# zacharielegault/lesion-gnn

Hardware: AMD Instinct MI355X
Metric: graphs/sec (fwd+bwd) on batched k-NN lesion graphs at 1/2/4/8 MI355X (higher is better)
Workload: dtype f32; 1 GPU; C2: 2-layer GCN fwd+CE+bwd+Adam, graph build per forward; step_launch=graph:step, criterion=CE fused with the model node (forward_loss), sync_bn=False, process_group=False, adam=lgnn, graphs_per_gpu=1024, global_batch=1024, nodes=65536, edges=524288, k=8, d_in=128, parallelism=dp1

## Files before the change

include/lgnn.h:

```cpp
#ifndef LGNN_H
#define LGNN_H

#include <stddef.h>
#include <stdint.h>

#ifdef __cplusplus
extern "C" {
#endif

#define LGNN_ABI_VERSION 40

#define LGNN_OK 0
#define LGNN_EINVAL (-22)
#define LGNN_ENOSPC (-28)
#define LGNN_EBUSY (-16)

#define LGNN_SLOT_FLAG0 7
#define LGNN_SLOT_FLAGS 256
#define LGNN_TILE_OPEN_EXTRA (LGNN_SLOT_FLAG0 + LGNN_SLOT_FLAGS)

#define LGNN_LOOPS_KEEP 0
#define LGNN_LOOPS_REMAINING 1
#define LGNN_LOOPS_READD 2

// ... 296 lines not shown
                               float* const* dWp, float* const* dbp, int num_partials,
                               float* dS_ws, int32_t* tile_open, const float* dlogits,
                               const float* Wout, int num_classes, const void* adjt,
                               void* stream);
struct lgnn_ce_src;
int lgnn_gcn_stack_bwd_s3f_ce(const int64_t* batch, const int32_t* gptr, int pool_mean,
                              int64_t num_graphs, const int32_t* rowptr, const int32_t* col,
                              const float* w, const int32_t* tptr, const int32_t* tidx,
                              const float* tw, const float* X, int64_t M, int L,
                              const uint16_t* planes_t, const float* const* W,
                              const float* const* H, const float* const* S, const int* widths,
                              float* const* dWp, float* const* dbp, int num_partials,
                              float* dS_ws, int32_t* tile_open, const struct lgnn_ce_src* ce,
                              const float* Wout, int num_classes, const void* adjt,
                              void* stream);

size_t lgnn_s3_weight_planes_numel(int out_features, int in_features, int planes);
int lgnn_s3_weight_planes(const float* W, int rows, int cols, int transposed, int planes,
                          uint16_t* Wp, void* stream);
#define LGNN_MAX_WPREP 16
int lgnn_s3_weight_planes_multi(int n, const float* const* W, const int* rows, const int* cols,
                                const int* transposed, int planes, uint16_t* const* Wp,
                                void* stream);
int lgnn_s3_gemm(const float* A, int64_t M, int K, const uint16_t* Wp, int N, int planes,
                 const float* bias, float* Y, float* colsum_part, void* stream);
int lgnn_s3_gemm_att(const float* A, int64_t M, int K, const uint16_t* Wp, int N, int planes,
                     float* Y, const float* att_src, const float* att_dst, int heads, int C,
                     float* a_s, float* a_d, void* stream);
int lgnn_s3_wgrad_partials(int64_t M, int K, int N);
int lgnn_s3_wgrad(const float* dY, int N, const float* X, int64_t M, int K, int planes,
// ... 165 lines not shown
```

lesion_gnn_amd/csrc/loss.hip:

```cpp
#include "common.h"

namespace {

constexpr int CT = 1024;

__device__ __forceinline__ float block_sum_fixed(float v, float* red) {
  const int lane = threadIdx.x & 63, wave = threadIdx.x >> 6;
  for (int o = 32; o > 0; o >>= 1) v += __shfl_xor(v, o, 64);
  if (lane == 0) red[wave] = v;
  __syncthreads();
  float t = 0.f;
  if (threadIdx.x == 0) {
    for (int w = 0; w < CT / 64; ++w) t += red[w];
    red[CT / 64] = t;
  }
  __syncthreads();
  return red[CT / 64];
}

template <bool FACTORS>
__global__ __launch_bounds__(CT) void k_ce_fwd(const float* __restrict__ z,
                                               const int64_t* __restrict__ y,
                                               const float* __restrict__ weight, int64_t B, int C,
                                               float* __restrict__ lse, float* __restrict__ loss,
// ... 87 lines not shown
  const float dl = smooth ? fminf(fmaxf(d, -1.f), 1.f) : 2.f * d;
  float g = gloss ? gloss[0] / (float)B * dl : 0.f;
  if (gpred) g += gpred[i];
  dz[i] = (zi >= lo && zi <= hi) ? g : 0.f;
}

struct ReduceJobs {
  CeSrc ce;
  int ce_part[LGNN_MAX_REDUCE];
  const float* part[LGNN_MAX_REDUCE];
  const float* factor[LGNN_MAX_REDUCE];
  float* out[LGNN_MAX_REDUCE];
  int64_t len[LGNN_MAX_REDUCE];
  int P[LGNN_MAX_REDUCE];
  int width[LGNN_MAX_REDUCE];
};

constexpr int RT = 1024;
__global__ __launch_bounds__(RT) void k_reduce_multi(ReduceJobs jobs) {
  __shared__ f32x4 red4[16][64];
  float(*red)[64] = reinterpret_cast<float(*)[64]>(red4);
  const int j = blockIdx.y;
  const int64_t len = jobs.len[j];
  const bool vec = !jobs.factor[j] && !jobs.ce_part[j] && (len & 3) == 0 && len >= 4096;
  if ((int64_t)blockIdx.x * (vec ? 256 : 64) >= len) return;
  const float* __restrict__ part = jobs.part[j];
  int P = jobs.P[j];
  const int lane = threadIdx.x & 63, wave = threadIdx.x >> 6;
  if (vec) {
    const int64_t i4 = (int64_t)blockIdx.x * 256 + 4 * lane;
    const int64_t ic4 = i4 < len ? i4 : len - 4;
    f32x4 s4 = {0.f, 0.f, 0.f, 0.f};
    int p = wave;
    for (; p + 16 * 15 < P; p += 16 * 16) {
      f32x4 v[16];
#pragma unroll
      for (int u = 0; u < 16; ++u) v[u] = ld4(part + (int64_t)(p + 16 * u) * len + ic4);
#pragma unroll
      for (int u = 0; u < 16; ++u) s4 += v[u];
    }
    for (; p < P; p += 16) s4 += ld4(part + (int64_t)p * len + ic4);
    red4[wave][lane] = s4;
    __syncthreads();
// ... 153 lines not shown
                       static_cast<const float*>(target), B, lo, hi, smooth_l1, grad_loss,
                       grad_pred, dz);
  LGNN_LAUNCH_CHECK();
  return LGNN_OK;
}

extern "C" int lgnn_reduce_partials_multi(int n, const float* const* partials,
                                          const int* num_partials, const int64_t* len,
                                          float* const* out, void* stream) {
  return lgnn_reduce_jobs(n, partials, nullptr, nullptr, num_partials, len, out, stream);
}

static int reduce_jobs(int n, const float* const* partials, const float* const* factor,
                       const int* width, const int* num_partials, const int64_t* len,
                       float* const* out, const int* ce_job, const lgnn_ce_src* ce, int C,
                       void* stream) {
  if (n <= 0 || n > LGNN_MAX_REDUCE || !partials || !num_partials || !len || !out)
    return LGNN_EINVAL;
  ReduceJobs jobs = {};
  if (ce_job) {
    if (!ce || !ce->pm || !ce->wt || !ce->wsum || !ce->gloss || C < 1)
      return LGNN_EINVAL;
    jobs.ce = CeSrc{ce->pm, ce->wt, ce->wsum, ce->gloss, C};
  }
  int64_t maxlen = 0;
  for (int j = 0; j < n; ++j) {
    const bool cj = ce_job && ce_job[j];
    if ((!partials[j] && !cj) || !out[j] || num_partials[j] <= 0 || len[j] < 0)
      return LGNN_EINVAL;
    if (cj) {
      const int64_t rows = factor && factor[j] && width ? len[j] / width[j] : len[j];
      if (rows != C) return LGNN_EINVAL;
      jobs.ce_part[j] = 1;
    }
    if (factor && factor[j]) {
      if (!width || width[j] <= 0 || len[j] % width[j] != 0) return LGNN_EINVAL;
      jobs.factor[j] = factor[j];
      jobs.width[j] = width[j];
    }
    jobs.part[j] = partials[j];
    jobs.out[j] = out[j];
    jobs.len[j] = len[j];
    jobs.P[j] = num_partials[j];
    if (len[j] > maxlen) maxlen = len[j];
  }
  if (maxlen == 0) return LGNN_OK;
  hipLaunchKernelGGL(k_reduce_multi, dim3((unsigned)((maxlen + 63) / 64), (unsigned)n), dim3(RT),
                     0, as_stream(stream), jobs);
  LGNN_LAUNCH_CHECK();
  return LGNN_OK;
}

extern "C" int lgnn_reduce_jobs(int n, const float* const* partials, const float* const* factor,
                                const int* width, const int* num_partials, const int64_t* len,
                                float* const* out, void* stream) {
  return reduce_jobs(n, partials, factor, width, num_partials, len, out, nullptr, nullptr, 0,
                     stream);
}

extern "C" int lgnn_reduce_jobs_ce(int n, const float* const* partials,
                                   const float* const* factor, const int* width,
                                   const int* num_partials, const int64_t* len,
                                   float* const* out, const int* ce_job, const lgnn_ce_src* ce,
                                   int num_classes, void* stream) {
  if (!ce_job) return LGNN_EINVAL;
  return reduce_jobs(n, partials, factor, width, num_partials, len, out, ce_job, ce, num_classes,
                     stream);
}
```

lesion_gnn_amd/csrc/node.hip:

```cpp
#include "common.h"
#include "tile.h"

namespace {

constexpr int TM = 64;
constexpr int TN = 128;
constexpr int KC = 128;
constexpr int LDS = KC + 4;
constexpr int NT = 256;
constexpr int CAPE = 1024;
constexpr int EB = 8;

struct TileIdx {
  int rp[TM + 1];
  int col[CAPE];
  float w[CAPE];
};

__device__ __forceinline__ f32x4 zero4() { return f32x4{0.f, 0.f, 0.f, 0.f}; }
__device__ __forceinline__ f32x4 sel4(bool c, f32x4 v) { return c ? v : zero4(); }

template <bool VEC>
__device__ __forceinline__ void fill_direct(float* Xs, const float* __restrict__ X, int64_t M,
                                            int K, int k0, int64_t r0) {
// ... 645 lines not shown
                                    H, act, X, M, K, rowptr, col, w, self_scale, W, N, dXpre,
                                    dW_partial, db_partial, num_partials, nullptr, 0, 0, stream);
}

extern "C" int lgnn_node_linear_bwd_tiles(int grad_mode, const float* dY, const int64_t* batch,
                                          const int32_t* gptr, int pool_mean,
                                          const int32_t* tptr, const int32_t* tidx,
                                          const float* tw, float tself, const float* H, int act,
                                          const float* X, int64_t M, int K,
                                          const int32_t* rowptr, const int32_t* col,
                                          const float* w, float self_scale, const float* W, int N,
                                          float* dXpre, float* dW_partial, float* db_partial,
                                          int num_partials, const int32_t* tile_open,
                                          int want_open, int accumulate, void* stream) {
  if (M < 0 || K <= 0 || N <= 0 || (N & 3) || !W || !dW_partial) return LGNN_EINVAL;
  if (accumulate < 0 || accumulate > 2 ||
      (accumulate == 2 && (!tile_open || num_partials > LGNN_SLOT_FLAGS)))
    return LGNN_EINVAL;
  const bool fast = bwd_fast(M, N, K, rowptr != nullptr);
  if (tile_open && !fast) return LGNN_EINVAL;
  if (!tile_open && num_partials != (fast ? lgnn_tile_partials(M) : grid_partials(M, N, K)))
    return LGNN_EINVAL;
  if (num_partials <= 0) return LGNN_EINVAL;
  if (act != LGNN_ACT_NONE && act != LGNN_ACT_ELU) return LGNN_EINVAL;
  if (act == LGNN_ACT_ELU && !H) return LGNN_EINVAL;
  if (grad_mode == LGNN_GRAD_POOL && (!batch || !gptr)) return LGNN_EINVAL;
  if (grad_mode == LGNN_GRAD_TRANSPOSE && (!tptr || !tidx)) return LGNN_EINVAL;
  if (grad_mode < 0 || grad_mode > 2 || (M > 0 && (!dY || !X))) return LGNN_EINVAL;
  const bool gather = rowptr != nullptr;
  if (gather && (!col || (K & 3))) return LGNN_EINVAL;
  if (fast && M > 0) {
    const hipError_t ef = lgnn_tile_bwd(s_(stream), grad_mode, dY, batch, gptr, pool_mean, tptr,
// ... 64 lines not shown
```

lesion_gnn_amd/csrc/stack3_bwd.hip:

```cpp
#include <cstdlib>
#include "common.h"
#include "tile.h"
#include "tile_util.h"
#include "s3_util.h"
#include "tile_lw.h"

namespace lgnn_s3 {

constexpr int BM_POOL = 0;
constexpr int BM_CONV = 1;
constexpr int BM_LIN = 2;

struct BwdLayerArgs {
  const float* dZin;
  const int64_t* batch;
  const int32_t* gptr;
  int pool_mean;
  int64_t num_graphs;
  const float* Hout;
  const float* Hin;
  const uint16_t* WpT;
  float* dZout;
  float* dWp;
  float* dbp;
// ... 572 lines not shown
        const float wgt = tw[j];
        const int64_t src = tidx[j];
        if (c < N) {
          a0 += wgt * dS[src * N + c];
          a1 += wgt * dS[src * N + c + 1];
        }
      }
      if (c < N) {
        dZ0[row * N + c] = a0;
        dZ0[row * N + c + 1] = a1;
      }
    }
  }
}

template <int NL, bool AG, bool XIN = false>
__global__ __launch_bounds__(NT, 1) void k_s3_fbwd(const int32_t* __restrict__ rowptr,
                                                   const int32_t* __restrict__ col,
                                                   const float* __restrict__ w, int64_t M,
                                                   FBwdArgs a, const int32_t* __restrict__ tmask,
                                                   OpenBwdArgs o) {
  constexpr int L = NL - 1;
  constexpr int ND = XIN ? NL - 1 : NL;
  __shared__ __attribute__((aligned(16))) FBwdSmem sm;
  const int64_t ntiles = (M + TM - 1) / TM;
  float* const scr = reinterpret_cast<float*>(sm.Adj[0]);
  const int NLast = a.width[L + 1];
  const Buf bP = mkbuf(a.dP, a.num_graphs * NLast * 4);

  f32x16 dw[ND][4];
#pragma unroll
  for (int l = 0; l < ND; ++l)
#pragma unroll
    for (int kb = 0; kb < 4; ++kb) dw[l][kb] = f32x16{};
  float dbacc[NL];
#pragma unroll
  for (int l = 0; l < NL; ++l) dbacc[l] = 0.f;

// ... 189 lines not shown
    if (has_next) idx_load_body(R, col, w);
    }
    const bool aexact = __builtin_amdgcn_readfirstlane(sm.flag) == 0;
    STAMP(stamp++);

    f32x16 xp[2];
#pragma unroll
    for (int l = L; l >= 1; --l) {
      const int K = a.width[l];
      const bool elu_prev = l >= 2;
      const bool fold = !XIN && l == 1;
      f32x16 hp[2];
      {
        const int tq = fresh_tid();
        const int h = (tq >> 5) & 1, k = 32 * (tq >> 6) + (tq & 31);
        load_pt(hp, a.H[l - 1], (ABL & 16) ? 0 : M, r0, K, k, K, h);
      }
      {
        float sacc = 0.f;
#pragma unroll
        for (int q = 0; q < 2; ++q)
#pragma unroll
          for (int r = 0; r < 16; ++r) sacc += dz[q][r];
        sacc += __shfl_xor(sacc, 32, 64);
        dbacc[l] += sacc;
      }
      u32x4 dzp[4][3];
      split_p(dz, dzp);
      if (fold && L == 1) {
        const int tq = fresh_tid();
        const int h = (tq >> 5) & 1, k = 32 * (tq >> 6) + (tq & 31);
// ... 55 lines not shown
      if (!fold) {
        const int tq = fresh_tid();
        const int h = (tq >> 5) & 1, li = tq & 31, wv = tq >> 6, qi = li & 3;
#pragma unroll
        for (int q = 0; q < 2; ++q)
#pragma unroll
          for (int j = 0; j < 4; ++j) {
            const int st = 2 * q + (j >> 1), i0 = 2 * (j & 1);
            const int off = ap_off(32 * q + 8 * j + 4 * h + qi, 32 * wv + (li & ~3));
#pragma unroll
            for (int p = 0; p < 3; ++p)
              sts8(sm.Gt[p] + off, quad_transpose_bf16(gp[st][p][i0], gp[st][p][i0 + 1], qi));
          }
      }
      STAMP(stamp++);
      {
        const int tq = fresh_tid();
        const int h = (tq >> 5) & 1, li = tq & 31, k = 32 * (tq >> 6) + li;
#pragma unroll
        for (int q = 0; q < 2; ++q)
#pragma unroll
          for (int gq = 0; gq < 4; ++gq) {
            u32x2 o[3];
            split4(f32x4{hp[q][4 * gq], hp[q][4 * gq + 1], hp[q][4 * gq + 2], hp[q][4 * gq + 3]},
                   o);
            const int off = hf_off(k, 32 * q + 8 * gq + 4 * h);
#pragma unroll
            for (int p = 0; p < 3; ++p) sts8(sm.Img[p] + off, o[p]);
          }
      }
      const uint16_t* wbase;
// ... 46 lines not shown
                nap = adj_split(sm);
              }
              const int t2 = fresh_tid();
              pre_cnt = (has_next && t2 < TM) ? a.gptr[pre_g + 1] - a.gptr[pre_g] : 0;
              if (has_head(a)) {
#pragma unroll
                for (int c = 0; c < kMaxHeadC; ++c)
                  pre_dl[c] = (has_next && t2 < TM && c < a.C) ? head_raw(a, pre_g, c) : 0.f;
                if (a.ce.pm) pre_wt = (has_next && t2 < TM) ? a.ce.wt[pre_g] : 0.f;
              }
            }
#pragma unroll
            for (int kb = 0; kb < 4; ++kb) {
              u32x4 hb[3], xb[3];
              const int off = hf_chunk(32 * kb + li, 2 * s + h);
#pragma unroll
              for (int p = 0; p < 3; ++p) hb[p] = lds16(sm.Img[p] + off);
#pragma unroll
              for (int p = 0; p < 3; ++p) xb[p] = lds16(sm.Gt[p] + off);
              if constexpr (!(ABL & 1)) {
                dw[1][kb] = mfma_s3(gp[s], hb, dw[1][kb]);
                dw[0][kb] = mfma_s3(gp[s], xb, dw[0][kb]);
              }
            }
            S3F_SB();
          }
        }
        lds_barrier();
        if constexpr (AG && kAdjPipe) {
          adj_write(sm, nap);
          lds_barrier();
        }
        STAMP(stamp++);
      } else {
      {
        const int tq = fresh_tid();
// ... 83 lines not shown
            pre_dl[c] = (has_next && tq < TM && c < a.C) ? head_raw(a, pre_g, c) : 0.f;
          if (a.ce.pm) pre_wt = (has_next && tq < TM) ? a.ce.wt[pre_g] : 0.f;
        }
      }
      lds_barrier();
      if constexpr (AG && kAdjPipe) {
        const AdjPlanes nap = adj_split(sm);
        lds_barrier();
        adj_write(sm, nap);
        lds_barrier();
      }
      STAMP(stamp++);
    }
    t = tn;
  }
  if (write_slots) {
    if constexpr (!XIN) {
      unsigned char* const timg = sm.Img[0];
      constexpr int TPL = 2 * TM * AROW;
      static_assert(3 * TPL == sizeof(sm.Img) + sizeof(sm.Gt) && offsetof(FBwdSmem, Gt) ==
                                                                     sizeof(sm.Img), "T image");
      float* const gl = sm.hl;
      lds_barrier();
      {
        const int tq = fresh_tid();
        const int h = (tq >> 5) & 1, li = tq & 31, wv = tq >> 6;
#pragma unroll
        for (int kb = 0; kb < 4; ++kb)
#pragma unroll
          for (int gq = 0; gq < 4; ++gq) {
            u32x2 o3[3];
            split4(f32x4{dw[0][kb][4 * gq], dw[0][kb][4 * gq + 1], dw[0][kb][4 * gq + 2],
// ... 53 lines not shown
        };
        fold_pair(wa, 0);
        load_w2(wa, 2);
        fold_pair(wb, 1);
        load_w2(wb, 3);
        fold_pair(wa, 2);
        fold_pair(wb, 3);
        dbs += __shfl_xor(dbs, 32, 64);
        dbacc[0] = dbs;
      }
      STAMP(stamp++);
    }
    const int tq = threadIdx.x;
    const int h = (tq >> 5) & 1, li = tq & 31, wv = tq >> 6;
#pragma unroll
    for (int l = XIN ? 1 : 0; l < NL; ++l) {
      const int N = a.width[l + 1], K = a.width[l];
      float* slab = a.dWp[l] + (int64_t)blockIdx.x * N * K;
#pragma unroll
      for (int kb = 0; kb < 4; ++kb) {
        const int k = 32 * kb + li;
#pragma unroll
        for (int r = 0; r < 16; ++r) {
          const int n = 32 * wv + (r & 3) + 8 * (r >> 2) + 4 * h;
          if (n < N && k < K) {
            st_wt(slab + (int64_t)n * K + k, dw[XIN ? l - 1 : l][kb][r]);
          }
        }
      }
      const int n = 32 * wv + li;
      if (h == 0 && n < N) a.dbp[l][(int64_t)blockIdx.x * N + n] = dbacc[l];
    }
  }
  if (o.sync && tmask[ntiles] > 0) {
    static_assert(sizeof(LwSmem) <= sizeof(FBwdSmem), "open-tile LDS aliases the fused LDS");
    __syncthreads();
    LwSmem& lw = *reinterpret_cast<LwSmem*>(&sm);
    for (int l = L; l >= 0; --l) {
      if (l < L) grid_sync(o.sync, L - l);
      const int K = a.width[l], N = a.width[l + 1];
      const float* Sx = l == 0 ? a.X : o.S[l - 1];
      if (l == L)
        bwd_tiles<LGNN_GRAD_POOL, LGNN_ACT_ELU, true>(
            lw.A, lw.C, lw.ti, a.dP, a.batch, a.gptr, a.pool_mean, nullptr, nullptr, nullptr, 0.f,
            a.H[l], Sx, M, K, o.W[l], N, o.dS[l & 1], a.dWp[l], a.dbp[l], tmask, 1, 1, a.dlog,
            a.Wout, a.C, BnFuse{}, a.ce);
      else if (l >= 1)
        bwd_tiles<LGNN_GRAD_TRANSPOSE, LGNN_ACT_ELU, true>(
            lw.A, lw.C, lw.ti, o.dS[(l + 1) & 1], a.batch, a.gptr, a.pool_mean, o.tptr, o.tidx,
            o.tw, 0.f, a.H[l], Sx, M, K, o.W[l], N, o.dS[l & 1], a.dWp[l], a.dbp[l], tmask, 1,
            1);
      else if constexpr (XIN)
        open_dz0(a.dZ0, o.dS[1], o.tptr, o.tidx, o.tw, M, N, tmask);
      else
        bwd_tiles<LGNN_GRAD_TRANSPOSE, LGNN_ACT_NONE, false>(
            lw.A, lw.C, lw.ti, o.dS[1], a.batch, a.gptr, a.pool_mean, o.tptr, o.tidx, o.tw, 0.f,
            nullptr, Sx, M, K, o.W[0], N, nullptr, a.dWp[0], a.dbp[0], tmask, 1, 1);
    }
    grid_exit(o.sync);
  }
}

}

static int stack_bwd_s3f(const float* dP, const int64_t* batch, const int32_t* gptr,
                         int pool_mean, int64_t num_graphs, const int32_t* rowptr,
                         const int32_t* col, const float* w, const float* X, int64_t M, int L,
                         const uint16_t* planes_t, const float* const* H, const int* widths,
                         float* const* dWp, float* const* dbp, int num_partials,
                         const int32_t* tile_open, const lgnn_s3::OpenBwdArgs& o, void* stream,
                         const float* dlogits = nullptr, const float* Wout = nullptr,
                         int num_classes = 0, const void* adjt = nullptr,
// ... 89 lines not shown
    if (dlogits || !ce->pm || !ce->wt || !ce->wsum || !ce->gloss)
      return LGNN_EINVAL;
    a.ce = CeSrc{ce->pm, ce->wt, ce->wsum, ce->gloss, num_classes};
  }
  a.Wout = Wout;
  a.C = num_classes;
  a.adjt = static_cast<const unsigned char*>(adjt);
  a.batch = batch;
  a.gptr = gptr;
  a.pool_mean = pool_mean;
  a.num_graphs = num_graphs;
  a.X = X;
  a.WpT = planes_t;
  a.dZ0 = dz0;
  for (int l = 0; l <= L + 1; ++l) a.width[l] = widths[l];
  for (int l = 0; l <= L; ++l) {
    if (!lgnn_tile_fits(M, widths[l], widths[l + 1]) || !H[l] || !dWp[l] || !dbp[l])
      return LGNN_EINVAL;
    a.H[l] = H[l];
    a.dWp[l] = dWp[l];
    a.dbp[l] = dbp[l];
  }
  hipStream_t s = as_stream(stream);
  if (M == 0) {
    for (int l = 0; l <= L; ++l)
      if (hipMemsetAsync(dWp[l], 0, (size_t)widths[l] * widths[l + 1] * 4, s) != hipSuccess ||
          hipMemsetAsync(dbp[l], 0, (size_t)widths[l + 1] * 4, s) != hipSuccess)
        return (int)hipGetLastError();
    return LGNN_OK;
  }
  const dim3 grid((unsigned)num_partials), blk(lgnn_tile::NT);
  if (o.sync) {
    const int cap = lgnn_fused_grid_capacity(1);
    if (cap < (int)grid.x) return cap == LGNN_EINVAL ? cap : cap < 0 ? -cap : LGNN_EBUSY;
  }
  if (L == 3 && adjt)
    hipLaunchKernelGGL((lgnn_s3::k_s3_fbwd<4, true, true>), grid, blk, 0, s, rowptr, col, w, M, a,
                       tile_open, o);
  else if (L == 3)
    hipLaunchKernelGGL((lgnn_s3::k_s3_fbwd<4, false, true>), grid, blk, 0, s, rowptr, col, w, M,
                       a, tile_open, o);
  else if (L == 1 && adjt)
    hipLaunchKernelGGL((lgnn_s3::k_s3_fbwd<2, true>), grid, blk, 0, s, rowptr, col, w, M, a,
                       tile_open, o);
  else if (L == 1)
    hipLaunchKernelGGL((lgnn_s3::k_s3_fbwd<2, false>), grid, blk, 0, s, rowptr, col, w, M, a,
                       tile_open, o);
  else if (adjt)
    hipLaunchKernelGGL((lgnn_s3::k_s3_fbwd<3, true>), grid, blk, 0, s, rowptr, col, w, M, a,
                       tile_open, o);
  else
    hipLaunchKernelGGL((lgnn_s3::k_s3_fbwd<3, false>), grid, blk, 0, s, rowptr, col, w, M, a,
                       tile_open, o);
  const hipError_t e = hipGetLastError();
  return e == hipSuccess ? LGNN_OK : (int)e;
}
// ... 12 lines not shown
```

lesion_gnn_amd/csrc/tile_lw.h:

```cpp
#pragma once
#include <type_traits>

#include "tile_util.h"

namespace lgnn_tile {

template <int UB = EB>
__device__ __forceinline__ f32x4 agg_row_local(const TileIdx& ti, int rr, const float* A) {
  static_assert(UB <= EB, "row batches read at most EB padding entries");
  const int li = threadIdx.x & 31;
  const int eb = ti.rp[0];
  const int e0 = ti.rp[rr] - eb, e1 = ti.rp[rr + 1] - eb;
  f32x4 acc = zero4();
  for (int e = e0; e < e1; e += UB) {
    int2 p[UB];
#pragma unroll
    for (int u = 0; u < UB; ++u) p[u] = ti.ow[e + u];
    f32x4 v[UB];
#pragma unroll
    for (int u = 0; u < UB; ++u) v[u] = ld4(A + p[u].x + 4 * li);
#pragma unroll
    for (int u = 0; u < UB; ++u) {
      const float wv = e + u < e1 ? __int_as_float(p[u].y) : 0.f;
      acc += wv * v[u];
// ... 450 lines not shown
#pragma unroll
              for (int j = 0; j < 4; ++j) {
                const float gg = v[j] * bn_elu_grad(z[j], bsc[j], bsh[j]) * m[j];
                const float xh = (z[j] - bmu[j]) * bis[j];
                s0[j] += (double)gg;
                s1[j] += (double)gg * (double)xh;
              }
            }
          }
        }
      }
    }
    __syncthreads();
  }
  if constexpr (BNM == BN_GSTATS) bn_part_write(reinterpret_cast<double*>(A), s0, s1, bn.part, K);
  const bool skipped = accumulate == 2 && blockIdx.x < LGNN_SLOT_FLAGS &&
                       tmask[ntiles + LGNN_SLOT_FLAG0 + blockIdx.x] != 0;
  if (accumulate && tfirst >= ntiles && !skipped) return;
  const bool add = accumulate && !skipped;
  float* slab = dWp + (int64_t)blockIdx.x * N * K;
#pragma unroll
  for (int j = 0; j < 4; ++j) {
    const int k = 32 * j + li;
#pragma unroll
    for (int r = 0; r < 16; ++r) {
      const int o = 32 * wave + (r & 3) + 8 * (r >> 2) + 4 * h;
      if (o < N && k < K) {
        float* p = slab + (int64_t)o * K + k;
        *p = add ? *p + dw[j][r] : dw[j][r];
      }
    }
  }
  if (dbp && tid < N) {
    float* p = dbp + (int64_t)blockIdx.x * N + tid;
    *p = add ? *p + dbacc : dbacc;
  }
}

}
```

lesion_gnn_amd/ops.py:

```python
from __future__ import annotations

import ctypes
import weakref
from collections import namedtuple
from typing import NamedTuple

import torch
from torch.utils import _pytree as pytree

from . import _lib
from .graph import NO_CSR, Csr, Graph


def _compiling() -> bool:
    return torch.compiler.is_compiling()


def _lgnn():
    from . import library

    return library


def _f32c(t: torch.Tensor) -> torch.Tensor:
# ... 40 lines not shown


STACK_MAX = 8


FUSED_BWD = True
LAZY_TRANSPOSE = True


MFMA_MODE = "s3"
BWD_MODE = "s3f"
BWD_S3 = BWD_MODE in ("s3", "s3f")
OPEN_IN_FUSED = "auto"
OPEN_IN_FUSED_BWD = OPEN_IN_FUSED
HEAD_FOLD = True
_CAPACITY: dict = {}


def fused_grid_capacity(direction: str, dev) -> int:
    key = (direction, torch.device(dev).index)
    cap = _CAPACITY.get(key)
    if cap is None:
        with torch.cuda.device(dev):
            cap = int(_lib.load().lgnn_fused_grid_capacity(0 if direction == "fwd" else 1))
        if cap < 0:
            _lib.check(cap, "lgnn_fused_grid_capacity")
        _CAPACITY[key] = cap
    return cap


# ... 132 lines not shown
        s_out = ss[l - 1] if l > 0 else None
        _lib.call("lgnn_node_linear_fwd_tiles", inp, M, inp.size(1), c.rowptr, c.col, c.w, 0.0,
                  Ws[l], bs[l], Ws[l].size(0),
                  _lib.LGNN_ACT_ELU if l > 0 else _lib.LGNN_ACT_NONE, hs[l], s_out, open_, 1,
                  _s(dev))
    return hs, ss, planes_t, adjt_t


def head_in_stack_bwd(graph: Graph, L: int, C: int, s3: bool) -> bool:
    return (HEAD_FOLD and s3 and BWD_MODE == "s3f" and L <= 3 and C <= 8 and
            _open_in_fused(OPEN_IN_FUSED_BWD, graph, "bwd"))


def stack_bwd(dp: torch.Tensor | None, x: torch.Tensor, graph: Graph, mean: bool, Ws: list,
              hs: list, ss: list, reducer: list, planes_t: torch.Tensor | None = None,
              head: tuple | None = None, kind: str = "gcn", adjt_t: torch.Tensor | None = None):
    csr = graph.csr(kind)
    open_ = graph.tile_open(kind)
    M = x.size(0)
    L = len(Ws) - 1
    dev = x.device
    lib = _lib.load()
    s3 = planes_t is not None
    s3f = s3 and _s3f(L) and (L <= 2 or _open_in_fused(OPEN_IN_FUSED_BWD, graph, "bwd"))
    adjt = (adjt_t if adjt_t is not None else _adjt_ptr(planes_t, L)) if s3f else None
    P = lib.lgnn_gcn_stack_bwd_s3_partials(M) if s3 and not s3f else \
        lib.lgnn_gcn_stack_bwd_partials(M)
    _lib.check(0 if P > 0 else P, "lgnn_gcn_stack_bwd_partials")
    widths = [x.size(1)] + [W.size(0) for W in Ws]
    per = [widths[l + 1] * widths[l] + widths[l + 1] for l in range(L + 1)]
    slab = torch.empty(P * sum(per), dtype=torch.float32, device=dev)
    dWp, dbp, off = [], [], 0
    for l in range(L + 1):
        nk, n = widths[l + 1] * widths[l], widths[l + 1]
        dWp.append(slab[off:off + P * nk])
        dbp.append(slab[off + P * nk:off + P * (nk + n)])
        off += P * (nk + n)
    Sx = [x] + list(ss)
    dlog, W_out = head if head is not None else (None, None)
    ce = dlog if isinstance(dlog, _lib.CeSrc) else None
    B = dp.size(0) if dp is not None else (graph.num_graphs if ce is not None else dlog.size(0))
    if s3f and _open_in_fused(OPEN_IN_FUSED_BWD, graph, "bwd"):
        dS_ws = torch.empty((3 if L == 3 else 2) * M * 128, dtype=torch.float32, device=dev)
        common = (graph.batch, graph.gptr, int(mean), B, csr.rowptr, csr.col, csr.w, csr.tptr,
                  csr.tidx, csr.tw, x, M, L, planes_t, Ws, hs, ss, widths, dWp, dbp, P, dS_ws,
                  open_)
        if ce is not None:
            _lib.call("lgnn_gcn_stack_bwd_s3f_ce", *common, ctypes.byref(ce), W_out,
                      W_out.size(0), adjt, _s(dev))
        else:
            _lib.call("lgnn_gcn_stack_bwd_s3f_all", dp, *common, dlog, W_out,
                      W_out.size(0) if head else 0, adjt, _s(dev))
        if L == 3:
            dz0 = dS_ws[2 * M * 128:2 * M * 128 + M * widths[1]].view(M, widths[1])
            first = dense_wgrad(dz0, x, False, want_db=True, reducer=reducer)
            return [first] + _stack_bwd_outputs(L, widths, dWp, dbp, P, dev, reducer, l0=1)
        return _stack_bwd_outputs(L, widths, dWp, dbp, P, dev, reducer)
    assert head is None, "dP from the logits gradient only in the single-launch split-3 path"
    if s3f:
        _lib.call("lgnn_gcn_stack_bwd_s3f", dp, graph.batch, graph.gptr, int(mean), dp.size(0),
                  csr.rowptr, csr.col, csr.w, x, M, L, planes_t, hs, widths, dWp, dbp, P, open_,
                  adjt, _s(dev))
    elif s3:
        dz_ws = torch.empty(2 * M * 128, dtype=torch.float32, device=dev)
        _lib.call("lgnn_gcn_stack_bwd_s3", dp, graph.batch, graph.gptr, int(mean), dp.size(0),
                  csr.rowptr, csr.col, csr.w, x, M, L, planes_t, hs, widths, dWp, dbp, P, dz_ws,
                  open_, _s(dev))
    else:
        _lib.call("lgnn_gcn_stack_bwd", dp, graph.batch, graph.gptr, int(mean), csr.rowptr,
                  csr.col, csr.w, x, M, L, Ws, hs, widths, dWp, dbp, P, open_, _s(dev))
    dS = None
    for l in reversed(range(L + 1)):
        K, N = widths[l], widths[l + 1]
        if l == L:
            mode, dY, tc = _lib.LGNN_GRAD_POOL, dp, NO_CSR
        else:
            mode, dY, tc = _lib.LGNN_GRAD_TRANSPOSE, dS, csr
        dX = torch.empty(M, K, dtype=torch.float32, device=dev) if l > 0 else None
        _lib.call("lgnn_node_linear_bwd_tiles", mode, dY, graph.batch, graph.gptr, int(mean),
                  tc.tptr, tc.tidx, tc.tw, 0.0, hs[l] if l > 0 else None,
                  _lib.LGNN_ACT_ELU if l > 0 else _lib.LGNN_ACT_NONE, Sx[l], M, K, None, None,
                  None, 0.0, Ws[l], N, dX, dWp[l], dbp[l], P, open_, 1, 2 if s3f else 1,
                  _s(dev))
        dS = dX
    return _stack_bwd_outputs(L, widths, dWp, dbp, P, dev, reducer)


def _stack_bwd_outputs(L, widths, dWp, dbp, P, dev, reducer, l0=0):
    out = []
    for l in range(l0, L + 1):
        dW = torch.empty(widths[l + 1], widths[l], dtype=torch.float32, device=dev)
        db = torch.empty(widths[l + 1], dtype=torch.float32, device=dev)
        reducer.extend([(dWp[l], P, dW.numel(), dW), (dbp[l], P, db.numel(), db)])
        out.append((dW, db))
    return out


def num_partials(M: int, N: int, K: int, gather: bool = False) -> int:
    p = _lib.load().lgnn_bwd_num_partials(M, N, K, int(gather))
    _lib.check(0 if p > 0 else p, "lgnn_bwd_num_partials")
# ... 47 lines not shown

CE_PART = object()


def reduce_multi(jobs: list, dev, ce=None, num_classes: int = 0) -> None:
    for i in range(0, len(jobs), 16):
        chunk = jobs[i:i + 16]
        n = len(chunk)
        is_ce = [j[0] is CE_PART for j in chunk]
        parts = [None if c else j[0] for j, c in zip(chunk, is_ce)]
        nps = [j[1] for j in chunk]
        lens = [j[2] for j in chunk]
        outs = [j[3] for j in chunk]
        fac = [j[4] if len(j) > 4 else None for j in chunk]
        wid = [j[5] if len(j) > 4 else 0 for j in chunk]
        if any(is_ce):
            if ce is None:
                raise _lib.LgnnError("reduce_multi: a CE_PART job needs the CE source")
            _lib.call("lgnn_reduce_jobs_ce", n, parts, fac, wid, nps, lens, outs,
                      [int(c) for c in is_ce], ctypes.byref(ce), int(num_classes), _s(dev))
        elif any(len(j) > 4 for j in chunk):
            _lib.call("lgnn_reduce_jobs", n, parts, fac, wid, nps, lens, outs, _s(dev))
        else:
            _lib.call("lgnn_reduce_partials_multi", n, parts, nps, lens, outs, _s(dev))


def spmm_raw(rowptr, col, w, self_scale: float, x: torch.Tensor) -> torch.Tensor:
    M, D = x.shape
    y = torch.empty_like(x)
    _lib.call("lgnn_spmm", rowptr, col, w, float(self_scale), x, M, D, y, _s(x.device))
    return y
# ... 523 lines not shown
    kind = sv.plan.kind
    csr = graph.csr(kind)
    W_out = params[2 + 2 * L]
    dlogits = _f32c(dlogits) if dlogits is not None else None
    grads = [None] * len(params)
    red: list = []
    if sv.plan.fused_bwd and not want_dx:
        Ws = [params[2 * l] for l in range(L + 1)]
        if head_in_stack_bwd(graph, L, W_out.size(0), sv.planes_t is not None):
            C, D = W_out.shape
            B = pooled.size(0)
            dWo = torch.empty_like(W_out)
            dbo = torch.empty(C, dtype=torch.float32, device=x.device)
            part = CE_PART if ce is not None else dlogits
            red += [(part, B, C * D, dWo, pooled, D), (part, B, C, dbo)]
            outs = stack_bwd(None, x, graph, sv.mean, Ws, hs, ss, red, sv.planes_t,
                             head=(ce[0] if ce is not None else dlogits, W_out), kind=kind,
                             adjt_t=sv.adjt)
        else:
            dp, dWo, dbo = pool_head_bwd(dlogits, pooled, W_out)
            outs = stack_bwd(dp, x, graph, sv.mean, Ws, hs, ss, red, sv.planes_t, kind=kind,
                             adjt_t=sv.adjt)
        grads[2 + 2 * L], grads[3 + 2 * L] = dWo, dbo
        for l, (dW, db) in enumerate(outs):
            grads[2 * l], grads[2 * l + 1] = dW, db
        reduce_multi(red, x.device, ce=ce[0] if ce is not None else None,
                     num_classes=W_out.size(0))
        return None, grads
    assert ce is None, "the CE-formed logits gradient only on the fused head path"
    dp, dWo, dbo = pool_head_bwd(dlogits, pooled, W_out)
    grads[2 + 2 * L], grads[3 + 2 * L] = dWo, dbo
    if sv.plan.fused:
        ss = [spmm_raw(csr.rowptr, csr.col, csr.w, 0.0, hs[l]) for l in range(L)]
    dS = None
    for l in reversed(range(L)):
        W = params[2 + 2 * l]
        if l == L - 1:
            mode, dY, tc = _lib.LGNN_GRAD_POOL, dp, None
        else:
            mode, dY, tc = _lib.LGNN_GRAD_TRANSPOSE, dS, csr
        saved_s = sv.plan.saved_s[l]
        dS, dW, db = linear_bwd(mode, dY, H=hs[l + 1], act=_lib.LGNN_ACT_ELU,
# ... 1447 lines not shown
```

Before: 4.891 million graphs/s.

## Defer in_proj/conv1 weight-grad fold into a post-reduce kernel for shallow GCN

For stacks with at most two conv layers and no saved H[0], the fused backward kernel stops forming the layer-1 weight gradient against H[0] per tile. It instead accumulates a compact T = dZ1ᵀ·X product plus a bias-gradient vector in extra partial slabs. A new fold kernel then reconstructs dW0, db0 and dW1 from T, W0, b0 and W1 once after the partial reduction, and a live flag lets the reduction skip or zero jobs. The aim is to drop the per-tile H[0] loads and MFMA work and to avoid materialising H[0]. The cost is an extra slab, an extra launch and more complex reduction and control logic.

After: 5.118 million graphs/s, median of 6. 4.6% higher.

```diff
diff --git a/include/lgnn.h b/include/lgnn.h
--- a/include/lgnn.h
+++ b/include/lgnn.h
@@ -334,6 +334,15 @@
                               float* dS_ws, int32_t* tile_open, const struct lgnn_ce_src* ce,
                               const float* Wout, int num_classes, const void* adjt,
                               void* stream);
+
+int lgnn_gcn_fold_wgrad(const float* T, const float* g, const float* W0, const float* b0,
+                        const float* W1, int d_in, int w1, int w2, const float* dW0_open,
+                        const float* db0_open, const float* dW1_open, const int32_t* live,
+                        float* dW0, float* db0, float* dW1, void* stream);
+int lgnn_reduce_jobs_live(int n, const float* const* partials, const float* const* factor,
+                          const int* width, const int* num_partials, const int64_t* len,
+                          float* const* out, const int* ce_job, const struct lgnn_ce_src* ce,
+                          int num_classes, const int32_t* const* live, void* stream);
 
 size_t lgnn_s3_weight_planes_numel(int out_features, int in_features, int planes);
 int lgnn_s3_weight_planes(const float* W, int rows, int cols, int transposed, int planes,
diff --git a/lesion_gnn_amd/csrc/foldgrad.hip b/lesion_gnn_amd/csrc/foldgrad.hip
--- /dev/null
+++ b/lesion_gnn_amd/csrc/foldgrad.hip
@@ -0,0 +1,153 @@
+#include "common.h"
+
+namespace {
+
+constexpr int FT = 256;
+constexpr int FR = 8;
+constexpr int FW = 128;
+constexpr int FLD = FW + 4;
+
+struct FoldArgs {
+  const float* T;
+  const float* g;
+  const float* W0;
+  const float* b0;
+  const float* W1;
+  const float* dW0_open;
+  const float* db0_open;
+  const float* dW1_open;
+  const int32_t* live;
+  float* dW0;
+  float* db0;
+  float* dW1;
+  int d_in, w1, w2;
+};
+
+__device__ __forceinline__ void copy_load(f32x4 (&v)[16], const float* src, int n4) {
+#pragma unroll
+  for (int u = 0; u < 16; ++u) {
+    const int f = threadIdx.x + u * FT;
+    v[u] = ld4(src + 4 * (int64_t)(f < n4 ? f : 0));
+  }
+}
+__device__ __forceinline__ void copy_store(float* dst, int ld, const f32x4 (&v)[16], int n4,
+                                           int q) {
+  int r = threadIdx.x / q, p = threadIdx.x - r * q;
+  const int dr = FT / q, dp = FT - dr * q;
+#pragma unroll
+  for (int u = 0; u < 16; ++u) {
+    if ((int)threadIdx.x + u * FT < n4) st4(dst + r * ld + 4 * p, v[u]);
+    r += dr;
+    p += dp;
+    if (p >= q) {
+      p -= q;
+      ++r;
+    }
+  }
+}
+
+__global__ __launch_bounds__(FT) void k_fold_wgrad(FoldArgs a) {
+  __shared__ __attribute__((aligned(16))) float big[FW * FLD];
+  __shared__ __attribute__((aligned(16))) float strip[FW * FR];
+  __shared__ float gs[FW];
+  const int t = threadIdx.x;
+  const int c = t & (FW - 1), rg = t >> 7;
+  const int d_in = a.d_in, w1 = a.w1, w2 = a.w2;
+  const int nb0 = (w1 + FR - 1) / FR;
+  const int q = d_in / 4;
+  const f32x4 z = {0.f, 0.f, 0.f, 0.f};
+  const bool role0 = (int)blockIdx.x < nb0;
+  const int r0 = FR * (role0 ? (int)blockIdx.x : (int)blockIdx.x - nb0);
+  const int rows = role0 ? w1 : w2, cols = role0 ? d_in : w1;
+  float* const out = role0 ? a.dW0 : a.dW1;
+  const float* const open = role0 ? a.dW0_open : a.dW1_open;
+  f32x4 v[16];
+  copy_load(v, role0 ? a.T : a.W0, (role0 ? w2 : w1) * q);
+  const bool alive = !a.live || a.live[0] != 0;
+  if (!alive && open == out && (!role0 || a.db0_open == a.db0)) return;
+  float ov[4] = {0.f, 0.f, 0.f, 0.f};
+  if (open && c < cols) {
+#pragma unroll
+    for (int j = 0; j < 4; ++j)
+      if (r0 + 4 * rg + j < rows) ov[j] = open[(int64_t)(r0 + 4 * rg + j) * cols + c];
+  }
+  const bool dbt = role0 && t < FR && r0 + t < w1;
+  const float obv = (a.db0_open && dbt) ? a.db0_open[r0 + t] : 0.f;
+  float acc[4] = {0.f, 0.f, 0.f, 0.f};
+  double dbs = 0.0;
+  if (alive) {
+    const float gv = t < w2 ? a.g[t] : 0.f;
+    if (role0) {
+      const int sn = t >> 1, si = r0 + 4 * (t & 1);
+      const f32x4 sv = (sn < w2 && si < w1) ? ld4(a.W1 + (int64_t)sn * w1 + si) : z;
+      copy_store(big, d_in, v, w2 * q, q);
+      st4(strip + FR * sn + 4 * (t & 1), sv);
+      if (t < FW) gs[t] = gv;
+      __syncthreads();
+      const int kc = c < d_in ? c : 0;
+#pragma unroll 8
+      for (int n = 0; n < w2; ++n) {
+        const float tv = big[n * d_in + kc];
+        const f32x4 wv = ld4(strip + FR * n + 4 * rg);
+#pragma unroll
+        for (int j = 0; j < 4; ++j) acc[j] = fmaf(wv[j], tv, acc[j]);
+      }
+      if (dbt) {
+        double s4[4] = {0.0, 0.0, 0.0, 0.0};
+        for (int n = 0; n < w2; n += 4) {
+#pragma unroll
+          for (int e = 0; e < 4; ++e)
+            s4[e] = fma((double)strip[FR * (n + e) + t], (double)gs[n + e], s4[e]);
+        }
+        dbs = (s4[0] + s4[1]) + (s4[2] + s4[3]);
+      }
+    } else {
+      const int sr = t / q, sp = t - sr * q;
+      const f32x4 sv =
+          (sr < FR && r0 + sr < w2) ? ld4(a.T + (int64_t)(r0 + sr) * d_in + 4 * sp) : z;
+      const float bv = c < w1 ? a.b0[c] : 0.f;
+      copy_store(big, FLD, v, w1 * q, q);
+      if (sr < FR) st4(strip + FW * sr + 4 * sp, sv);
+      if (t < FW) gs[t] = gv;
+      __syncthreads();
+      const int ic = c < w1 ? c : 0;
+#pragma unroll 4
+      for (int p = 0; p < q; ++p) {
+        const f32x4 wv = ld4(big + ic * FLD + 4 * p);
+#pragma unroll
+        for (int j = 0; j < 4; ++j) {
+          const f32x4 tv = ld4(strip + FW * (4 * rg + j) + 4 * p);
+#pragma unroll
+          for (int e = 0; e < 4; ++e) acc[j] = fmaf(tv[e], wv[e], acc[j]);
+        }
+      }
+#pragma unroll
+      for (int j = 0; j < 4; ++j) acc[j] = fmaf(gs[(r0 + 4 * rg + j) & (FW - 1)], bv, acc[j]);
+    }
+  }
+  if (c < cols) {
+#pragma unroll
+    for (int j = 0; j < 4; ++j) {
+      const int r = r0 + 4 * rg + j;
+      if (r < rows) out[(int64_t)r * cols + c] = open ? acc[j] + ov[j] : acc[j];
+    }
+  }
+  if (dbt) a.db0[r0 + t] = (float)(a.db0_open ? dbs + (double)obv : dbs);
+}
+
+}
+
+extern "C" int lgnn_gcn_fold_wgrad(const float* T, const float* g, const float* W0,
+                                   const float* b0, const float* W1, int d_in, int w1, int w2,
+                                   const float* dW0_open, const float* db0_open,
+                                   const float* dW1_open, const int32_t* live, float* dW0,
+                                   float* db0, float* dW1, void* stream) {
+  if (!T || !g || !W0 || !b0 || !W1 || !dW0 || !db0 || !dW1) return LGNN_EINVAL;
+  for (const int w : {d_in, w1, w2})
+    if (w < 4 || w > FW || w % 4 != 0) return LGNN_EINVAL;
+  FoldArgs a = {T, g, W0, b0, W1, dW0_open, db0_open, dW1_open, live, dW0, db0, dW1, d_in, w1, w2};
+  const unsigned grid = (unsigned)((w1 + FR - 1) / FR + (w2 + FR - 1) / FR);
+  hipLaunchKernelGGL(k_fold_wgrad, dim3(grid), dim3(FT), 0, as_stream(stream), a);
+  LGNN_LAUNCH_CHECK();
+  return LGNN_OK;
+}
diff --git a/lesion_gnn_amd/csrc/loss.hip b/lesion_gnn_amd/csrc/loss.hip
--- a/lesion_gnn_amd/csrc/loss.hip
+++ b/lesion_gnn_amd/csrc/loss.hip
@@ -125,6 +125,7 @@
   int64_t len[LGNN_MAX_REDUCE];
   int P[LGNN_MAX_REDUCE];
   int width[LGNN_MAX_REDUCE];
+  const int32_t* live[LGNN_MAX_REDUCE];
 };
 
 constexpr int RT = 1024;
@@ -138,6 +139,18 @@
   const float* __restrict__ part = jobs.part[j];
   int P = jobs.P[j];
   const int lane = threadIdx.x & 63, wave = threadIdx.x >> 6;
+  if (const int32_t* lv = jobs.live[j]; lv && *lv == 0) {
+    if (wave == 0) {
+      if (vec) {
+        const int64_t i4 = (int64_t)blockIdx.x * 256 + 4 * lane;
+        if (i4 < len) st4(jobs.out[j] + i4, f32x4{0.f, 0.f, 0.f, 0.f});
+      } else {
+        const int64_t i = (int64_t)blockIdx.x * 64 + lane;
+        if (i < len) jobs.out[j][i] = 0.f;
+      }
+    }
+    return;
+  }
   if (vec) {
     const int64_t i4 = (int64_t)blockIdx.x * 256 + 4 * lane;
     const int64_t ic4 = i4 < len ? i4 : len - 4;
@@ -321,7 +334,7 @@
 static int reduce_jobs(int n, const float* const* partials, const float* const* factor,
                        const int* width, const int* num_partials, const int64_t* len,
                        float* const* out, const int* ce_job, const lgnn_ce_src* ce, int C,
-                       void* stream) {
+                       void* stream, const int32_t* const* live = nullptr) {
   if (n <= 0 || n > LGNN_MAX_REDUCE || !partials || !num_partials || !len || !out)
     return LGNN_EINVAL;
   ReduceJobs jobs = {};
@@ -349,6 +362,7 @@
     jobs.out[j] = out[j];
     jobs.len[j] = len[j];
     jobs.P[j] = num_partials[j];
+    jobs.live[j] = live ? live[j] : nullptr;
     if (len[j] > maxlen) maxlen = len[j];
   }
   if (maxlen == 0) return LGNN_OK;
@@ -374,3 +388,13 @@
   return reduce_jobs(n, partials, factor, width, num_partials, len, out, ce_job, ce, num_classes,
                      stream);
 }
+
+extern "C" int lgnn_reduce_jobs_live(int n, const float* const* partials,
+                                     const float* const* factor, const int* width,
+                                     const int* num_partials, const int64_t* len,
+                                     float* const* out, const int* ce_job, const lgnn_ce_src* ce,
+                                     int num_classes, const int32_t* const* live, void* stream) {
+  if (!live) return LGNN_EINVAL;
+  return reduce_jobs(n, partials, factor, width, num_partials, len, out, ce_job, ce, num_classes,
+                     stream, live);
+}
diff --git a/lesion_gnn_amd/csrc/node.hip b/lesion_gnn_amd/csrc/node.hip
--- a/lesion_gnn_amd/csrc/node.hip
+++ b/lesion_gnn_amd/csrc/node.hip
@@ -683,8 +683,8 @@
                                           int num_partials, const int32_t* tile_open,
                                           int want_open, int accumulate, void* stream) {
   if (M < 0 || K <= 0 || N <= 0 || (N & 3) || !W || !dW_partial) return LGNN_EINVAL;
-  if (accumulate < 0 || accumulate > 2 ||
-      (accumulate == 2 && (!tile_open || num_partials > LGNN_SLOT_FLAGS)))
+  if (accumulate < 0 || accumulate > 4 || (accumulate >= 3 && !tile_open) ||
+      ((accumulate == 2 || accumulate == 4) && (!tile_open || num_partials > LGNN_SLOT_FLAGS)))
     return LGNN_EINVAL;
   const bool fast = bwd_fast(M, N, K, rowptr != nullptr);
   if (tile_open && !fast) return LGNN_EINVAL;
diff --git a/lesion_gnn_amd/csrc/stack3_bwd.hip b/lesion_gnn_amd/csrc/stack3_bwd.hip
--- a/lesion_gnn_amd/csrc/stack3_bwd.hip
+++ b/lesion_gnn_amd/csrc/stack3_bwd.hip
@@ -610,7 +610,7 @@
   }
 }
 
-template <int NL, bool AG, bool XIN = false>
+template <int NL, bool AG, bool XIN = false, bool DF = false>
 __global__ __launch_bounds__(NT, 1) void k_s3_fbwd(const int32_t* __restrict__ rowptr,
                                                    const int32_t* __restrict__ col,
                                                    const float* __restrict__ w, int64_t M,
@@ -618,6 +618,7 @@
                                                    OpenBwdArgs o) {
   constexpr int L = NL - 1;
   constexpr int ND = XIN ? NL - 1 : NL;
+  static_assert(!DF || (!XIN && NL <= 3), "deferred fold: in_proj folded behind the first conv");
   __shared__ __attribute__((aligned(16))) FBwdSmem sm;
   const int64_t ntiles = (M + TM - 1) / TM;
   float* const scr = reinterpret_cast<float*>(sm.Adj[0]);
@@ -837,7 +838,7 @@
       {
         const int tq = fresh_tid();
         const int h = (tq >> 5) & 1, k = 32 * (tq >> 6) + (tq & 31);
-        load_pt(hp, a.H[l - 1], (ABL & 16) ? 0 : M, r0, K, k, K, h);
+        if (!(DF && fold)) load_pt(hp, a.H[l - 1], (ABL & 16) ? 0 : M, r0, K, k, K, h);
       }
       {
         float sacc = 0.f;
@@ -923,7 +924,7 @@
           }
       }
       STAMP(stamp++);
-      {
+      if (!(DF && fold)) {
         const int tq = fresh_tid();
         const int h = (tq >> 5) & 1, li = tq & 31, k = 32 * (tq >> 6) + li;
 #pragma unroll
@@ -1000,12 +1001,14 @@
             for (int kb = 0; kb < 4; ++kb) {
               u32x4 hb[3], xb[3];
               const int off = hf_chunk(32 * kb + li, 2 * s + h);
-#pragma unroll
-              for (int p = 0; p < 3; ++p) hb[p] = lds16(sm.Img[p] + off);
+              if constexpr (!DF) {
+#pragma unroll
+                for (int p = 0; p < 3; ++p) hb[p] = lds16(sm.Img[p] + off);
+              }
 #pragma unroll
               for (int p = 0; p < 3; ++p) xb[p] = lds16(sm.Gt[p] + off);
               if constexpr (!(ABL & 1)) {
-                dw[1][kb] = mfma_s3(gp[s], hb, dw[1][kb]);
+                if constexpr (!DF) dw[1][kb] = mfma_s3(gp[s], hb, dw[1][kb]);
                 dw[0][kb] = mfma_s3(gp[s], xb, dw[0][kb]);
               }
             }
@@ -1119,8 +1122,28 @@
     }
     t = tn;
   }
+  const int closed_tiles = DF ? (int)ntiles - tmask[ntiles] : 0;
+  if (DF && blockIdx.x == 0 && threadIdx.x == 0)
+    *reinterpret_cast<int32_t*>(a.dbp[NL] + (int64_t)gridDim.x * a.width[2]) = closed_tiles;
+  if (DF && closed_tiles > 0) {
+    const int tq = threadIdx.x;
+    const int h = (tq >> 5) & 1, li = tq & 31, wv = tq >> 6;
+    const int N = a.width[2], K = a.width[0];
+    float* slab = a.dWp[NL] + (int64_t)blockIdx.x * N * K;
+#pragma unroll
+    for (int kb = 0; kb < 4; ++kb) {
+      const int k = 32 * kb + li;
+#pragma unroll
+      for (int r = 0; r < 16; ++r) {
+        const int n = 32 * wv + (r & 3) + 8 * (r >> 2) + 4 * h;
+        if (n < N && k < K) st_wt(slab + (int64_t)n * K + k, dw[0][kb][r]);
+      }
+    }
+    const int n = 32 * wv + li;
+    if (h == 0 && n < N) a.dbp[NL][(int64_t)blockIdx.x * N + n] = dbacc[0];
+  }
   if (write_slots) {
-    if constexpr (!XIN) {
+    if constexpr (!XIN && !DF) {
       unsigned char* const timg = sm.Img[0];
       constexpr int TPL = 2 * TM * AROW;
       static_assert(3 * TPL == sizeof(sm.Img) + sizeof(sm.Gt) && offsetof(FBwdSmem, Gt) ==
@@ -1204,11 +1227,11 @@
     const int tq = threadIdx.x;
     const int h = (tq >> 5) & 1, li = tq & 31, wv = tq >> 6;
 #pragma unroll
-    for (int l = XIN ? 1 : 0; l < NL; ++l) {
+    for (int l = (XIN || DF) ? 1 : 0; l < NL; ++l) {
       const int N = a.width[l + 1], K = a.width[l];
       float* slab = a.dWp[l] + (int64_t)blockIdx.x * N * K;
 #pragma unroll
-      for (int kb = 0; kb < 4; ++kb) {
+      for (int kb = 0; kb < (DF && l == 1 ? 0 : 4); ++kb) {
         const int k = 32 * kb + li;
 #pragma unroll
         for (int r = 0; r < 16; ++r) {
@@ -1230,22 +1253,23 @@
       if (l < L) grid_sync(o.sync, L - l);
       const int K = a.width[l], N = a.width[l + 1];
       const float* Sx = l == 0 ? a.X : o.S[l - 1];
+      const int dw1_acc = (DF && l == 1) ? 3 : 1;
       if (l == L)
         bwd_tiles<LGNN_GRAD_POOL, LGNN_ACT_ELU, true>(
             lw.A, lw.C, lw.ti, a.dP, a.batch, a.gptr, a.pool_mean, nullptr, nullptr, nullptr, 0.f,
-            a.H[l], Sx, M, K, o.W[l], N, o.dS[l & 1], a.dWp[l], a.dbp[l], tmask, 1, 1, a.dlog,
+            a.H[l], Sx, M, K, o.W[l], N, o.dS[l & 1], a.dWp[l], a.dbp[l], tmask, 1, dw1_acc, a.dlog,
             a.Wout, a.C, BnFuse{}, a.ce);
       else if (l >= 1)
         bwd_tiles<LGNN_GRAD_TRANSPOSE, LGNN_ACT_ELU, true>(
             lw.A, lw.C, lw.ti, o.dS[(l + 1) & 1], a.batch, a.gptr, a.pool_mean, o.tptr, o.tidx,
             o.tw, 0.f, a.H[l], Sx, M, K, o.W[l], N, o.dS[l & 1], a.dWp[l], a.dbp[l], tmask, 1,
-            1);
+            dw1_acc);
       else if constexpr (XIN)
         open_dz0(a.dZ0, o.dS[1], o.tptr, o.tidx, o.tw, M, N, tmask);
       else
         bwd_tiles<LGNN_GRAD_TRANSPOSE, LGNN_ACT_NONE, false>(
             lw.A, lw.C, lw.ti, o.dS[1], a.batch, a.gptr, a.pool_mean, o.tptr, o.tidx, o.tw, 0.f,
-            nullptr, Sx, M, K, o.W[0], N, nullptr, a.dWp[0], a.dbp[0], tmask, 1, 1);
+            nullptr, Sx, M, K, o.W[0], N, nullptr, a.dWp[0], a.dbp[0], tmask, 1, DF ? 0 : 1);
     }
     grid_exit(o.sync);
   }
@@ -1365,12 +1389,19 @@
   a.WpT = planes_t;
   a.dZ0 = dz0;
   for (int l = 0; l <= L + 1; ++l) a.width[l] = widths[l];
+  const bool defer = L <= 2 && !H[0];
   for (int l = 0; l <= L; ++l) {
-    if (!lgnn_tile_fits(M, widths[l], widths[l + 1]) || !H[l] || !dWp[l] || !dbp[l])
+    if (!lgnn_tile_fits(M, widths[l], widths[l + 1]) || (!H[l] && !(defer && l == 0)) ||
+        !dWp[l] || !dbp[l])
       return LGNN_EINVAL;
     a.H[l] = H[l];
     a.dWp[l] = dWp[l];
     a.dbp[l] = dbp[l];
+  }
+  if (defer) {
+    if (!dWp[L + 1] || !dbp[L + 1]) return LGNN_EINVAL;
+    a.dWp[L + 1] = dWp[L + 1];
+    a.dbp[L + 1] = dbp[L + 1];
   }
   hipStream_t s = as_stream(stream);
   if (M == 0) {
@@ -1378,6 +1409,11 @@
       if (hipMemsetAsync(dWp[l], 0, (size_t)widths[l] * widths[l + 1] * 4, s) != hipSuccess ||
           hipMemsetAsync(dbp[l], 0, (size_t)widths[l + 1] * 4, s) != hipSuccess)
         return (int)hipGetLastError();
+    if (defer && (hipMemsetAsync(dWp[L + 1], 0, (size_t)widths[2] * widths[0] * 4, s) != hipSuccess ||
+                  hipMemsetAsync(dbp[L + 1], 0, (size_t)widths[2] * 4, s) != hipSuccess ||
+                  hipMemsetAsync(dbp[L + 1] + (size_t)num_partials * widths[2], 0, 4, s) !=
+                      hipSuccess))
+      return (int)hipGetLastError();
     return LGNN_OK;
   }
   const dim3 grid((unsigned)num_partials), blk(lgnn_tile::NT);
@@ -1391,6 +1427,18 @@
   else if (L == 3)
     hipLaunchKernelGGL((lgnn_s3::k_s3_fbwd<4, false, true>), grid, blk, 0, s, rowptr, col, w, M,
                        a, tile_open, o);
+  else if (defer && L == 1 && adjt)
+    hipLaunchKernelGGL((lgnn_s3::k_s3_fbwd<2, true, false, true>), grid, blk, 0, s, rowptr, col,
+                       w, M, a, tile_open, o);
+  else if (defer && L == 1)
+    hipLaunchKernelGGL((lgnn_s3::k_s3_fbwd<2, false, false, true>), grid, blk, 0, s, rowptr, col,
+                       w, M, a, tile_open, o);
+  else if (defer && adjt)
+    hipLaunchKernelGGL((lgnn_s3::k_s3_fbwd<3, true, false, true>), grid, blk, 0, s, rowptr, col,
+                       w, M, a, tile_open, o);
+  else if (defer)
+    hipLaunchKernelGGL((lgnn_s3::k_s3_fbwd<3, false, false, true>), grid, blk, 0, s, rowptr, col,
+                       w, M, a, tile_open, o);
   else if (L == 1 && adjt)
     hipLaunchKernelGGL((lgnn_s3::k_s3_fbwd<2, true>), grid, blk, 0, s, rowptr, col, w, M, a,
                        tile_open, o);
diff --git a/lesion_gnn_amd/csrc/tile_lw.h b/lesion_gnn_amd/csrc/tile_lw.h
--- a/lesion_gnn_amd/csrc/tile_lw.h
+++ b/lesion_gnn_amd/csrc/tile_lw.h
@@ -488,10 +488,13 @@
     __syncthreads();
   }
   if constexpr (BNM == BN_GSTATS) bn_part_write(reinterpret_cast<double*>(A), s0, s1, bn.part, K);
-  const bool skipped = accumulate == 2 && blockIdx.x < LGNN_SLOT_FLAGS &&
+  const bool dw_over = accumulate >= 3;
+  const int acc = dw_over ? accumulate - 2 : accumulate;
+  const bool skipped = acc == 2 && blockIdx.x < LGNN_SLOT_FLAGS &&
                        tmask[ntiles + LGNN_SLOT_FLAG0 + blockIdx.x] != 0;
-  if (accumulate && tfirst >= ntiles && !skipped) return;
-  const bool add = accumulate && !skipped;
+  const bool leave = acc && tfirst >= ntiles && !skipped;
+  if (leave && !dw_over) return;
+  const bool add = acc && !skipped;
   float* slab = dWp + (int64_t)blockIdx.x * N * K;
 #pragma unroll
   for (int j = 0; j < 4; ++j) {
@@ -501,11 +504,11 @@
       const int o = 32 * wave + (r & 3) + 8 * (r >> 2) + 4 * h;
       if (o < N && k < K) {
         float* p = slab + (int64_t)o * K + k;
-        *p = add ? *p + dw[j][r] : dw[j][r];
-      }
-    }
-  }
-  if (dbp && tid < N) {
+        *p = (add && !dw_over) ? *p + dw[j][r] : dw[j][r];
+      }
+    }
+  }
+  if (dbp && tid < N && !leave) {
     float* p = dbp + (int64_t)blockIdx.x * N + tid;
     *p = add ? *p + dbacc : dbacc;
   }
diff --git a/lesion_gnn_amd/ops.py b/lesion_gnn_amd/ops.py
--- a/lesion_gnn_amd/ops.py
+++ b/lesion_gnn_amd/ops.py
@@ -78,6 +78,7 @@
 OPEN_IN_FUSED = "auto"
 OPEN_IN_FUSED_BWD = OPEN_IN_FUSED
 HEAD_FOLD = True
+DEFER_FOLD = True
 _CAPACITY: dict = {}
 
 
@@ -240,7 +241,8 @@
 
 def stack_bwd(dp: torch.Tensor | None, x: torch.Tensor, graph: Graph, mean: bool, Ws: list,
               hs: list, ss: list, reducer: list, planes_t: torch.Tensor | None = None,
-              head: tuple | None = None, kind: str = "gcn", adjt_t: torch.Tensor | None = None):
+              head: tuple | None = None, kind: str = "gcn", adjt_t: torch.Tensor | None = None,
+              b0: torch.Tensor | None = None):
     csr = graph.csr(kind)
     open_ = graph.tile_open(kind)
     M = x.size(0)
@@ -255,10 +257,15 @@
     _lib.check(0 if P > 0 else P, "lgnn_gcn_stack_bwd_partials")
     widths = [x.size(1)] + [W.size(0) for W in Ws]
     per = [widths[l + 1] * widths[l] + widths[l + 1] for l in range(L + 1)]
-    slab = torch.empty(P * sum(per), dtype=torch.float32, device=dev)
+    defer = DEFER_FOLD and s3f and L <= 2 and b0 is not None
+    if defer:
+        per.append(widths[2] * widths[0] + widths[2])
+        hs = [None] + list(hs[1:])
+    slab = torch.empty(P * sum(per) + int(defer), dtype=torch.float32, device=dev)
     dWp, dbp, off = [], [], 0
-    for l in range(L + 1):
-        nk, n = widths[l + 1] * widths[l], widths[l + 1]
+    for l in range(L + 2 if defer else L + 1):
+        nk, n = (widths[2] * widths[0], widths[2]) if l == L + 1 else \
+            (widths[l + 1] * widths[l], widths[l + 1])
         dWp.append(slab[off:off + P * nk])
         dbp.append(slab[off + P * nk:off + P * (nk + n)])
         off += P * (nk + n)
@@ -280,8 +287,11 @@
         if L == 3:
             dz0 = dS_ws[2 * M * 128:2 * M * 128 + M * widths[1]].view(M, widths[1])
             first = dense_wgrad(dz0, x, False, want_db=True, reducer=reducer)
-            return [first] + _stack_bwd_outputs(L, widths, dWp, dbp, P, dev, reducer, l0=1)
-        return _stack_bwd_outputs(L, widths, dWp, dbp, P, dev, reducer)
+            return [first] + _stack_bwd_outputs(L, widths, dWp, dbp, P, dev, reducer, l0=1), None
+        if defer:
+            return _stack_bwd_outputs_defer(L, widths, dWp, dbp, P, dev, reducer, Ws, b0, open_,
+                                            M, slab)
+        return _stack_bwd_outputs(L, widths, dWp, dbp, P, dev, reducer), None
     assert head is None, "dP from the logits gradient only in the single-launch split-3 path"
     if s3f:
         _lib.call("lgnn_gcn_stack_bwd_s3f", dp, graph.batch, graph.gptr, int(mean), dp.size(0),
@@ -306,10 +316,37 @@
         _lib.call("lgnn_node_linear_bwd_tiles", mode, dY, graph.batch, graph.gptr, int(mean),
                   tc.tptr, tc.tidx, tc.tw, 0.0, hs[l] if l > 0 else None,
                   _lib.LGNN_ACT_ELU if l > 0 else _lib.LGNN_ACT_NONE, Sx[l], M, K, None, None,
-                  None, 0.0, Ws[l], N, dX, dWp[l], dbp[l], P, open_, 1, 2 if s3f else 1,
-                  _s(dev))
+                  None, 0.0, Ws[l], N, dX, dWp[l], dbp[l], P, open_, 1,
+                  ((0, 4)[l] if l < 2 else 2) if defer else 2 if s3f else 1, _s(dev))
         dS = dX
-    return _stack_bwd_outputs(L, widths, dWp, dbp, P, dev, reducer)
+    if defer:
+        return _stack_bwd_outputs_defer(L, widths, dWp, dbp, P, dev, reducer, Ws, b0, open_, M,
+                                        slab)
+    return _stack_bwd_outputs(L, widths, dWp, dbp, P, dev, reducer), None
+
+
+def _stack_bwd_outputs_defer(L, widths, dWp, dbp, P, dev, reducer, Ws, b0, open_, M, slab):
+    d_in, w1, w2 = widths[0], widths[1], widths[2]
+    live = open_[(M + 63) // 64:]
+    closed = slab[-1:].view(torch.int32)
+    T = torch.empty(w2, d_in, dtype=torch.float32, device=dev)
+    g = torch.empty(w2, dtype=torch.float32, device=dev)
+    out = []
+    for l in range(L + 1):
+        dW = torch.empty(widths[l + 1], widths[l], dtype=torch.float32, device=dev)
+        db = torch.empty(widths[l + 1], dtype=torch.float32, device=dev)
+        reducer.extend([(dWp[l], P, dW.numel(), dW, None, 0, live if l < 2 else None),
+                        (dbp[l], P, db.numel(), db, None, 0, live if l < 1 else None)])
+        out.append((dW, db))
+    reducer.extend([(dWp[L + 1], P, T.numel(), T, None, 0, closed),
+                    (dbp[L + 1], P, g.numel(), g, None, 0, closed)])
+    (dW0, db0), dW1 = out[0], out[1][0]
+
+    def fold():
+        _lib.call("lgnn_gcn_fold_wgrad", T, g, Ws[0], b0, Ws[1], d_in, w1, w2, dW0, db0, dW1,
+                  closed, dW0, db0, dW1, _s(dev))
+
+    return out, fold
 
 
 def _stack_bwd_outputs(L, widths, dWp, dbp, P, dev, reducer, l0=0):
@@ -387,7 +424,15 @@
         outs = [j[3] for j in chunk]
         fac = [j[4] if len(j) > 4 else None for j in chunk]
         wid = [j[5] if len(j) > 4 else 0 for j in chunk]
-        if any(is_ce):
+        live = [j[6] if len(j) > 6 else None for j in chunk]
+        if any(lv is not None for lv in live):
+            if any(is_ce) and ce is None:
+                raise _lib.LgnnError("reduce_multi: a CE_PART job needs the CE source")
+            _lib.call("lgnn_reduce_jobs_live", n, parts, fac, wid, nps, lens, outs,
+                      [int(c) for c in is_ce] if any(is_ce) else None,
+                      ctypes.byref(ce) if any(is_ce) else None, int(num_classes), live,
+                      _s(dev))
+        elif any(is_ce):
             if ce is None:
                 raise _lib.LgnnError("reduce_multi: a CE_PART job needs the CE source")
             _lib.call("lgnn_reduce_jobs_ce", n, parts, fac, wid, nps, lens, outs,
@@ -941,18 +986,20 @@
             dbo = torch.empty(C, dtype=torch.float32, device=x.device)
             part = CE_PART if ce is not None else dlogits
             red += [(part, B, C * D, dWo, pooled, D), (part, B, C, dbo)]
-            outs = stack_bwd(None, x, graph, sv.mean, Ws, hs, ss, red, sv.planes_t,
-                             head=(ce[0] if ce is not None else dlogits, W_out), kind=kind,
-                             adjt_t=sv.adjt)
+            outs, after = stack_bwd(None, x, graph, sv.mean, Ws, hs, ss, red, sv.planes_t,
+                                    head=(ce[0] if ce is not None else dlogits, W_out),
+                                    kind=kind, adjt_t=sv.adjt, b0=params[1])
         else:
             dp, dWo, dbo = pool_head_bwd(dlogits, pooled, W_out)
-            outs = stack_bwd(dp, x, graph, sv.mean, Ws, hs, ss, red, sv.planes_t, kind=kind,
-                             adjt_t=sv.adjt)
+            outs, after = stack_bwd(dp, x, graph, sv.mean, Ws, hs, ss, red, sv.planes_t,
+                                    kind=kind, adjt_t=sv.adjt, b0=params[1])
         grads[2 + 2 * L], grads[3 + 2 * L] = dWo, dbo
         for l, (dW, db) in enumerate(outs):
             grads[2 * l], grads[2 * l + 1] = dW, db
         reduce_multi(red, x.device, ce=ce[0] if ce is not None else None,
                      num_classes=W_out.size(0))
+        if after is not None:
+            after()
         return None, grads
     assert ce is None, "the CE-formed logits gradient only on the fused head path"
     dp, dWo, dbo = pool_head_bwd(dlogits, pooled, W_out)
```
